# sqeazy/sqeazy

Hardware: AMD Instinct MI355X
Metric: encode GB/s (input voxels) for bitswap1->lz4 uint16 volume (higher is better)
Workload: dtype u16

## Files before the change

sqeazy_amd/csrc/sqy_capi.cpp:

```cpp
#include "../../include/sqeazy_amd.h"

#include <hip/hip_runtime.h>

#include <algorithm>
#include <chrono>
#include <climits>
#include <cstdint>
#include <cstdio>
#include <cstdlib>
#include <cstring>
#include <atomic>
#include <condition_variable>
#include <memory>
#include <mutex>
#include <string>
#include <thread>
#include <vector>

#include "sqy_kernels.h"
#include "sqy_lanes.hpp"
#include "sqy_pipeline.hpp"

namespace {

// ... 17 lines not shown
    const char* v = std::getenv(name);
    if (!v || !*v) return dflt;
    char* end = nullptr;
    const long long x = std::strtoll(v, &end, 10);
    if (*end != '\0' || x < lo || x > hi) {
        std::fprintf(stderr, "[sqeazy]\t %s=%s is not a number in [%ld, %ld]: ignored\n", name, v, lo, hi);
        return dflt;
    }
    return (long)x;
}
constexpr long kWarmupMax = 1l << 30;
constexpr long kStageLanesDefault = 2, kParseLanesDefault = 3;
constexpr long kBatchBytesMax = (1l << 32) - 1, kBatchGroupBytesDefault = 1l << 30;
constexpr long kBatchJointMaxDefault = 128l << 20;
struct Options {
    std::atomic<long> transpose_chain;
    std::atomic<long> transpose_chain_caller_streams;
    std::atomic<long> block_parallel;
    std::atomic<long> block_parallel_warmup;
    std::atomic<long> block_parallel_stats;
    std::atomic<long> tail_scan;
    std::atomic<long> decode_two_waves;
    std::atomic<long> noise_digest;
    std::atomic<long> transpose_blocks_per_cu;
    std::atomic<long> stored_tail_index;
    std::atomic<long> host_l2_bytes;
    std::atomic<long> decode_frames_subset;
    std::atomic<long> decode_slabs_joint;
    std::atomic<long> encode_batch_joint;
    std::atomic<long> encode_batch_group_bytes;
    std::atomic<long> encode_batch_joint_max_bytes;
    std::atomic<long> stage_lanes;
    std::atomic<long> parse_lanes;
    std::atomic<long> lane_calls{0}, lane_backlog_fallbacks{0}, lane_blocked_fallbacks{0};
    std::atomic<long> call_stamps{0};
    Options()
        : transpose_chain(env_flag("SQY_NO_TRANSPOSE_CHAIN") ? 0 : 1), transpose_chain_caller_streams(env_flag("SQY_TRANSPOSE_CHAIN_CALLER_STREAMS")),
          block_parallel(env_flag("SQY_NO_BLOCK_PARALLEL") ? 0 : 1), block_parallel_warmup(env_number("SQY_BLOCK_PARALLEL_WARMUP", 65536, 0, kWarmupMax)),
          block_parallel_stats(env_flag("SQY_BLOCK_PARALLEL_STATS")), tail_scan(env_flag("SQY_NO_TAIL_SCAN") ? 0 : 1),
          decode_two_waves(env_flag("SQY_NO_DECODE_TWO_WAVES") ? 0 : 1), noise_digest(env_flag("SQY_NO_NOISE_DIGEST") ? 0 : 1),
          transpose_blocks_per_cu(env_number("SQY_TRANSPOSE_BLOCKS_PER_CU", 32, 1, 64)), stored_tail_index(env_flag("SQY_NO_STORED_TAIL_INDEX") ? 0 : 1),
          host_l2_bytes((long)sqy::host_l2_cache_bytes()), decode_frames_subset(env_flag("SQY_NO_DECODE_FRAMES_SUBSET") ? 0 : 1),
          decode_slabs_joint(env_flag("SQY_NO_DECODE_SLABS_JOINT") ? 0 : 1), encode_batch_joint(env_flag("SQY_NO_ENCODE_BATCH_JOINT") ? 0 : 1),
          encode_batch_group_bytes(env_number("SQY_ENCODE_BATCH_GROUP_BYTES", kBatchGroupBytesDefault, 1, kBatchBytesMax)),
          encode_batch_joint_max_bytes(env_number("SQY_ENCODE_BATCH_JOINT_MAX_BYTES", kBatchJointMaxDefault, 0, kBatchBytesMax)), stage_lanes(env_number("SQY_STAGE_LANES", kStageLanesDefault, 0, 2)),
          parse_lanes(env_number("SQY_PARSE_LANES", kParseLanesDefault, 1, sqy::LanePicker::kMaxLanes)) { sqy::set_bitswap1_blocks_per_cu(transpose_blocks_per_cu.load()); }
    std::atomic<long>* find(const char* name)
    {
        if (!name) return nullptr;
        if (!std::strcmp(name, "transpose_chain")) return &transpose_chain;
        if (!std::strcmp(name, "transpose_chain_caller_streams")) return &transpose_chain_caller_streams;
        if (!std::strcmp(name, "block_parallel")) return &block_parallel;
        if (!std::strcmp(name, "block_parallel_warmup")) return &block_parallel_warmup;
        if (!std::strcmp(name, "block_parallel_stats")) return &block_parallel_stats;
        if (!std::strcmp(name, "tail_scan")) return &tail_scan;
        if (!std::strcmp(name, "decode_two_waves")) return &decode_two_waves;
        if (!std::strcmp(name, "noise_digest")) return &noise_digest;
        if (!std::strcmp(name, "transpose_blocks_per_cu")) return &transpose_blocks_per_cu;
        if (!std::strcmp(name, "stored_tail_index")) return &stored_tail_index;
        if (!std::strcmp(name, "host_l2_bytes")) return &host_l2_bytes;
        if (!std::strcmp(name, "decode_frames_subset")) return &decode_frames_subset;
        if (!std::strcmp(name, "decode_slabs_joint")) return &decode_slabs_joint;
        if (!std::strcmp(name, "encode_batch_joint")) return &encode_batch_joint;
        if (!std::strcmp(name, "encode_batch_group_bytes")) return &encode_batch_group_bytes;
        if (!std::strcmp(name, "encode_batch_joint_max_bytes")) return &encode_batch_joint_max_bytes;
        if (!std::strcmp(name, "stage_lanes")) return &stage_lanes;
        if (!std::strcmp(name, "parse_lanes")) return &parse_lanes;
        if (!std::strcmp(name, "lane_calls")) return &lane_calls;
        if (!std::strcmp(name, "lane_backlog_fallbacks")) return &lane_backlog_fallbacks;
        if (!std::strcmp(name, "lane_blocked_fallbacks")) return &lane_blocked_fallbacks;
        if (!std::strcmp(name, "call_stamps")) return &call_stamps;
        return nullptr;
    }
};
Options g_opt;

struct CallStamps {
    enum { entry, lanes_taken, clear_launched, transpose_launched, parse_queued, sync_returned, returned, kStamps };
    long seq = -1;
    long lane = -1;
    long thread = 0;
    long ns[kStamps] = {};
    void stamp(int i) { ns[i] = (long)std::chrono::duration_cast<std::chrono::nanoseconds>(std::chrono::steady_clock::now().time_since_epoch()).count(); }
};
constexpr size_t kStampRing = 8192;
std::mutex g_stamps_mu;
std::vector<CallStamps> g_stamps;
size_t g_stamps_next = 0;
struct StampScope {
    CallStamps rec;
    const bool on;
    StampScope() : on(g_opt.call_stamps.load(std::memory_order_relaxed) != 0) 
    {
        if (!on) return;
        rec.stamp(CallStamps::entry);
        rec.thread = (long)(std::hash<std::thread::id>()(std::this_thread::get_id()) & 0x7fffffff);
    }
    CallStamps* get() { return on ? &rec : nullptr; }
    ~StampScope()
    {
// ... 109 lines not shown
    {
        if (bytes <= cap) return 0;
        if (p) { hipHostFree(p); p = nullptr; cap = 0; }
        const size_t want = (bytes + ((size_t)1 << 16) - 1) & ~(((size_t)1 << 16) - 1);
        if (hipHostMalloc(&p, want, hipHostMallocDefault) != hipSuccess) {
            std::fprintf(stderr, "[sqeazy]\t unable to allocate %zu bytes of pinned host memory\n", want);
            (void)hipGetLastError();
            p = nullptr;
            return 1;
        }
        cap = want;
        return 0;
    }
    void release() { if (p) hipHostFree(p); p = nullptr; cap = 0; }
};

struct Workspace {
    DevBuf ping, pong, lz4_scratch, csize, frame_off, io_src, io_dst, small, plan, dedupe;
    DevBuf spec;
    DevBuf diff_side;
    DevBuf digest;
    DevBuf bkrd;
    DevBuf subset;
    DevBuf range_full;
    DevBuf slabs_index;
    DevBuf slabs_joint;
    DevBuf slabs_out;
    HostBuf slabs_host;
    DevBuf batch_stream;
    DevBuf batch_scratch;
    DevBuf batch_tables;
    HostBuf batch_host;
    void* pinned = nullptr;
    void release_buffers()
    {
        ping.release(); pong.release(); lz4_scratch.release(); csize.release(); frame_off.release();
        io_src.release(); io_dst.release(); small.release(); plan.release(); dedupe.release(); diff_side.release(); spec.release(); digest.release(); bkrd.release();
        subset.release(); range_full.release(); slabs_index.release(); slabs_joint.release(); slabs_out.release(); slabs_host.release();
        batch_stream.release(); batch_scratch.release(); batch_tables.release(); batch_host.release();
    }
};

struct Stager {
    static constexpr int kLanes = 4;
    static constexpr size_t kSlice = 8u << 20;
    char* pin[kLanes][2] = {};
    hipStream_t st[kLanes] = {};
    hipEvent_t ev[kLanes][2] = {};
    bool ready = false;

    bool init()
    {
        if (ready) return true;
        for (int l = 0; l < kLanes; ++l) {
            if (hipStreamCreateWithFlags(&st[l], hipStreamNonBlocking) != hipSuccess) return false;
            for (int b = 0; b < 2; ++b) {
                if (hipHostMalloc((void**)&pin[l][b], kSlice, hipHostMallocDefault) != hipSuccess) return false;
                if (hipEventCreateWithFlags(&ev[l][b], hipEventDisableTiming) != hipSuccess) return false;
            }
        }
        ready = true;
        return true;
    }
    bool copy(void* dev, void* host, size_t bytes, bool to_device, int device_id)
    {
        if (bytes == 0) return true;
        if (!init()) return false;
        const size_t nslices = (bytes + kSlice - 1) / kSlice;
// ... 219 lines not shown
Lz4Descriptor lz4_descriptor(int block_id)
{
    const unsigned char fd[2] = {0x40, (unsigned char)(block_id << 4)};
    return {fd[0], fd[1], (sqy::xxh32(fd, 2, 0) >> 8) & 0xff};
}

struct EncodeCall {
    Context& cx;
    Workspace* ws;
    std::vector<PendingEvent>* pend;
    hipStream_t stream;
    LaneLease* lanes;
    CallStamps* stamps;
    Pipeline pipe;
    std::vector<uint64_t> dims;
    uint64_t len;
    int elem_size;
    void* d_dst;
    uint64_t dst_capacity;
    long* dstoffset;
    FrameQuery* fq;

    const uint8_t* cur;
    int cur_elem;
    uint64_t cur_len;
    bool use_ping = true;

    struct {
        sqy::Lz4DedupeLayout dedupe;
        sqy::Lz4InplacePlan place;
        uint32_t* digest = nullptr;
        uint32_t digest_stride = 0;
        bool dedupe_cleared = false;
        const uint64_t* frame_map = nullptr;
        uint64_t frame_bytes = 0;
    } prep;
    struct DiffSide { const uint16_t* p = nullptr; uint32_t w = 0, X = 0; } side;
    struct {
        bool on = false;
        int block_id = 0;
        uint64_t total = 0, chunk = 0, nchunks = 0, stride = 0;
        const sqy::Lz4Block* blocks = nullptr;
        const uint32_t* dup_of = nullptr;
        uint64_t* tail_info = nullptr;
        bool inplace_done = false;
        uint64_t blob_at = 0, blob_bytes = 0, payload_bytes = 0;
    } lz4;

    EncodeCall(Context& c, hipStream_t s, Pipeline&& p, std::vector<uint64_t>&& d, uint64_t voxels, int elem, const void* src, void* dst,
               uint64_t capacity, long* offset, FrameQuery* frames, LaneLease* lane_lease, CallStamps* call_stamps)
        : cx(c), ws(&c.ws), pend(&c.pending), stream(s), lanes(lane_lease), stamps(call_stamps), pipe(std::move(p)), dims(std::move(d)), len(voxels), elem_size(elem), d_dst(dst),
          dst_capacity(capacity), dstoffset(offset), fq(frames), cur(static_cast<const uint8_t*>(src)), cur_elem(elem), cur_len(voxels) {}

    uint8_t* next_buf(size_t bytes)
    {
        DevBuf& b = use_ping ? ws->ping : ws->pong;
        use_ping = !use_ping;
        return b.ensure(bytes) ? nullptr : static_cast<uint8_t*>(b.p);
    }
    int produced(const uint8_t* out) { cur = out; return 0; }
    bool is_tail(size_t si) const { return pipe.sink_index >= 0 && (int)si > pipe.sink_index; }
    bool not_3d(const char* scheme) const
    {
        if (dims.size() != 3) std::fprintf(stderr, "[sqeazy::detail::%s::encode] received non-3D shape which is currently unsupported!\n", scheme);
        return dims.size() != 3;
    }
    bool followed_by(size_t si, StageKind k) const { return si + 1 < pipe.stages.size() && pipe.stages[si + 1].kind == k; }
    void stage_shape(size_t si, uint64_t& Z, uint64_t& Y, uint64_t& X) const
    {
        const bool flat = is_tail(si) && cur_len * (uint64_t)cur_elem != len;
        Z = flat ? 1 : dims[0]; Y = flat ? 1 : dims[1]; X = flat ? cur_len : dims[2];
    }

    int take_lanes(std::unique_lock<std::mutex>& lock)
    {
        const long mode = g_opt.stage_lanes.load();
        if (!lanes || mode == 0 || (mode == 2 && !g_opt.transpose_chain_caller_streams.load()) || (stream != nullptr && stream == cx.stream)) return 0;
        int devid = 0;
        if (hipGetDevice(&devid) != hipSuccess || devid < 0 || devid >= kMaxDev) return 0;
        if (!cx.ensure_lane_event()) { std::fprintf(stderr, "[sqeazy]\t no HIP event for the lanes\n"); return 1; }
        const auto deadline = std::chrono::steady_clock::now() + kLaneArrival;
        for (;;) {
            const hipError_t e = hipStreamQuery(stream);
            if (e == hipSuccess) break;
            (void)hipGetLastError();
// ... 66 lines not shown
            SQY_HIP(hipStreamWaitEvent(stream, g_tchain_last[devid], 0));
        g_tchain_when[devid] = now;
        tc.devid = devid;
        return 0;
    }
    int chain_record(TransposeChain& tc)
    {
        if (tc.devid < 0) return 0;
        SQY_HIP(hipEventRecord(cx.t_done, stream));
        g_tchain_last[tc.devid] = cx.t_done;
        tc.lock.unlock();
        return 0;
    }

    int bitswap1_for_lz4(size_t si, std::unique_lock<std::mutex>& lane_lock)
    {
        const sqy::Lz4Params& lz = pipe.stages[si + 1].lz4;
        const sqy::Lz4EncodeLayout lay = sqy::lz4_encode_layout(lz, cur_len * 2, pipe.nthreads);
        const uint64_t words = sqy::bitswap1_piece_hash_words(cur, cur, cur_len);
        prep.dedupe = sqy::lz4_dedupe_layout(lay, words);
        if (!prep.dedupe.total) return 0;
        if (ws->dedupe.ensure(prep.dedupe.total)) return 1;
        const uint64_t hdr_max = sqy::header_pack(elem_size, false, dims, pipe.name(), (uint64_t)INT_MAX).size() + 2;
        prep.place = sqy::lz4_inplace_plan(lay, words, si + 2 == pipe.stages.size(), dstoffset != nullptr,
                                           (unsigned)(reinterpret_cast<uintptr_t>(d_dst) & 15), dst_capacity, hdr_max);
        if (!prep.place.on) return 0;
        if (ws->plan.ensure((lay.nchunks + 1) * sizeof(uint32_t))) return 1;
        const uint32_t dstride = sqy::lz4_noise_digest_words(lz, lay, g_opt.noise_digest.load() != 0, cur_len / 8);
        if (dstride && !ws->digest.ensure(lay.nchunks * (uint64_t)dstride * sizeof(uint32_t), true)) {
            prep.digest = static_cast<uint32_t*>(ws->digest.p);
            prep.digest_stride = dstride;
        }
        if (take_lanes(lane_lock)) return 1;
        SQY_HIP(sqy::launch_lz4_dedupe_clear(ws->dedupe.p, prep.dedupe, static_cast<uint32_t*>(ws->plan.p), stream));
        prep.dedupe_cleared = true;
        if (stamps) stamps->stamp(CallStamps::clear_launched);
        return 0;
    }

    int bitswap1(size_t si)
    {
        std::unique_lock<std::mutex> lane_lock;
        if (cur_elem == 2 && followed_by(si, StageKind::lz4) && bitswap1_for_lz4(si, lane_lock)) return 1;
        const bool inplace = prep.place.on;
        uint8_t* out = inplace ? static_cast<uint8_t*>(d_dst) + prep.place.body0 : next_buf(cur_len * cur_elem);
        if (!out) return 1;
        if (!inplace && (reinterpret_cast<uintptr_t>(out) & 15)) prep.dedupe = sqy::Lz4DedupeLayout();
        uint32_t* ph = prep.dedupe.total ? static_cast<uint32_t*>(ws->dedupe.p) : nullptr;
        const bool on_lanes = lanes && lanes->taken();
        TransposeChain tc;
        if (chain_wait(tc, inplace)) return 1;
        if (cur_elem == 2)
            SQY_TIMED("bitswap1_u16", sqy::launch_bitswap1_u16(reinterpret_cast<const uint16_t*>(cur), reinterpret_cast<uint16_t*>(out), cur_len, stream, ph,
                                                               inplace ? (uint32_t)prep.place.chunk : 0, side.p, side.w, side.X, inplace ? prep.digest : nullptr,
                                                               prep.digest_stride));
        else
            SQY_TIMED("bitswap1_u8", sqy::launch_bitswap1_u8(cur, out, cur_len, stream));
        if (chain_record(tc)) return 1;
        if (stamps) stamps->stamp(CallStamps::transpose_launched);
        if (on_lanes && leave_transpose_lane(lane_lock)) return 1;
        side = DiffSide();
        return produced(out);
    }

    int reorder(size_t si, bool zcurve)
    {
        const char* name = zcurve ? "zcurve_reorder" : "raster_reorder";
// ... 252 lines not shown
                                           prep.dedupe_cleared, fused_dedupe ? &dedupe_args : nullptr));
            lz4.dup_of = reinterpret_cast<const uint32_t*>(static_cast<const uint8_t*>(ws->dedupe.p) + prep.dedupe.dup_at);
            if (fused_dedupe && prep.digest) { dedupe_args.digest = prep.digest; dedupe_args.digest_stride = prep.digest_stride; }
        }
        if (ws->plan.ensure((lz4.nchunks + 1) * sizeof(uint32_t))) return 1;
        uint32_t* d_redo = static_cast<uint32_t*>(ws->plan.p);
        SQY_TIMED("lz4_chunks", sqy::launch_lz4_chunks(cur, lz4.total, (uint32_t)lz4.chunk, static_cast<uint8_t*>(ws->lz4_scratch.p), lz4.stride,
                                                       static_cast<uint32_t*>(ws->csize.p), lz4.nchunks, stream, prep.frame_map, prep.frame_bytes, d_redo,
                                                       fused_dedupe ? nullptr : lz4.dup_of, prep.place.in_stride, accel, prep.dedupe_cleared,
                                                       fused_dedupe ? &dedupe_args : nullptr));
        std::string hdr_prefix, hdr_suffix;
        if (prep.place.on && !(fq && fq->every > 0)) sqy::header_pack_parts(elem_size, false, dims, pipe.name(), &hdr_prefix, &hdr_suffix);
        if (prep.place.on && !hdr_prefix.empty() && hdr_prefix.size() + hdr_suffix.size() <= sqy::kLz4InplaceHeaderTextMax)
            return lz4_inplace_finish(d_redo, hdr_prefix, hdr_suffix);
        SQY_HIP(hipMemcpyAsync(ws->pinned, d_redo, sizeof(uint32_t), hipMemcpyDeviceToHost, stream));
        SQY_HIP(hipStreamSynchronize(stream));
        const uint32_t n_redo = *static_cast<uint32_t*>(ws->pinned);
        return n_redo ? lz4_dense(d_redo, n_redo) : 0;
    }

    int lz4_dense(uint32_t* d_redo, uint32_t n_redo)
    {
        SQY_TIMED("lz4_chunks_dense", sqy::launch_lz4_chunks_dense(cur, lz4.total, (uint32_t)lz4.chunk, static_cast<uint8_t*>(ws->lz4_scratch.p), lz4.stride,
                                                                   static_cast<uint32_t*>(ws->csize.p), d_redo, n_redo, stream, prep.frame_map, prep.frame_bytes,
                                                                   prep.place.in_stride));
        return 0;
    }

    int lz4_inplace_finish(uint32_t* d_redo, const std::string& hdr_prefix, const std::string& hdr_suffix)
    {
        const Lz4Descriptor fd = lz4_descriptor(lz4.block_id);
        uint8_t* outb = static_cast<uint8_t*>(d_dst);
        volatile uint64_t* record = static_cast<volatile uint64_t*>(ws->pinned);
        const bool fused_tail = lz4.nchunks <= 65536;
        auto tail = [&](const uint32_t* guard, bool fused, bool scan_too) -> int {
            record[0] = 0;
            if (!fused && scan_too)
                SQY_TIMED("lz4_frame_scan", sqy::launch_lz4_frame_scan(static_cast<uint32_t*>(ws->csize.p), lz4.nchunks, lz4.total, (uint32_t)lz4.chunk,
                                                                       static_cast<uint64_t*>(ws->frame_off.p), stream, nullptr, lz4.dup_of, lz4.tail_info, guard,
                                                                       outb + prep.place.body0, prep.place.in_stride, fd.bd, fd.hc));
            auto with_args = [&](auto launch) {
                return launch(outb, prep.place.t0, prep.place.in_stride, lz4.total, (uint32_t)lz4.chunk, lz4.nchunks, static_cast<uint8_t*>(ws->lz4_scratch.p), lz4.stride,
                              static_cast<uint32_t*>(ws->csize.p), static_cast<uint64_t*>(ws->frame_off.p), lz4.dup_of, lz4.tail_info, fd.bd, fd.hc,
                              hdr_prefix.data(), (uint32_t)hdr_prefix.size(), hdr_suffix.data(), (uint32_t)hdr_suffix.size(), (uint32_t)elem_size, guard,
                              const_cast<uint64_t*>(record), stream);
            };
            SQY_TIMED(fused ? "lz4_inplace_tail" : "lz4_frame_gather",
                      fused ? with_args(sqy::launch_lz4_inplace_tail_fused) : with_args(sqy::launch_lz4_inplace_tail));
            return 0;
        };
        if (tail(d_redo, fused_tail, true)) return 1;
        if (stamps) stamps->stamp(CallStamps::parse_queued);
        SQY_HIP(hipStreamSynchronize(stream));
        if (stamps) stamps->stamp(CallStamps::sync_returned);
        if (record[0] == 2) {
            if (lz4_dense(d_redo, (uint32_t)record[6])) return 1;
            if (tail(nullptr, fused_tail, true)) return 1;
            SQY_HIP(hipStreamSynchronize(stream));
        }
        if (record[0] == 4) {
            if (tail(nullptr, false, false)) return 1;
            SQY_HIP(hipStreamSynchronize(stream));
        }
        if (record[0] != 1) {
            std::fprintf(stderr, "[sqeazy]\t internal error: frames in place did not finish (status %llu)\n", (unsigned long long)record[0]);
            return 1;
        }
        lz4.inplace_done = true;
        lz4.blob_at = record[1]; lz4.blob_bytes = record[2]; lz4.payload_bytes = record[3];
        lz4.on = true;
        return 0;
    }

    int lz4_linked(size_t si, bool serial, uint32_t accel)
    {
        const sqy::Lz4Plan plan = sqy::lz4_plan_blocks(lz4.total, lz4.chunk, pipe.stages[si].lz4.block_bytes(), serial);
        if (!plan.ok || plan.blocks.empty()) {
            std::fprintf(stderr, "[sqeazy]\t lz4: block layout not available on MI355X\n");
            return 1;
        }
        const uint64_t nblocks = plan.blocks.size(), nframes = plan.frame_first.size() - 1;
        const uint64_t blocks_bytes = nblocks * sizeof(sqy::Lz4Block), first_bytes = (nframes + 1) * sizeof(uint32_t);
        static_assert(sizeof(sqy::Lz4Block) == sizeof(sqy::Lz4BlockPlan) && sizeof(sqy::Lz4Block) == 32, "plan entries are read by the kernels as they are");
        if (ws->plan.ensure(blocks_bytes + first_bytes)) return 1;
        sqy::Lz4Block* d_blocks = static_cast<sqy::Lz4Block*>(ws->plan.p);
        uint32_t* d_first = reinterpret_cast<uint32_t*>(static_cast<uint8_t*>(ws->plan.p) + blocks_bytes);
        SQY_HIP(hipMemcpyAsync(d_blocks, plan.blocks.data(), blocks_bytes, hipMemcpyHostToDevice, stream));
// ... 139 lines not shown
        if (tail.j) {
            SQY_TIMED("lz4_frame_gather", sqy::launch_lz4_frame_gather(body0, lz4.total, (uint32_t)lz4.chunk, static_cast<uint8_t*>(ws->lz4_scratch.p), lz4.stride,
                                                                       static_cast<uint32_t*>(ws->csize.p), static_cast<uint64_t*>(ws->frame_off.p), out + payload_at, fd.bd, fd.hc,
                                                                       tail.j, stream, nullptr, 0, nullptr, lz4.dup_of, prep.place.in_stride, tail.raw_head != 0));
        }
        SQY_HIP(hipMemcpyAsync(out + *blob_at, hdr.data(), hdr.size(), hipMemcpyHostToDevice, stream));
        SQY_HIP(hipStreamSynchronize(stream));
        return 0;
    }

    int assemble_plain(const std::string& hdr, uint64_t payload_bytes)
    {
        uint8_t* out = static_cast<uint8_t*>(d_dst);
        const Lz4Descriptor fd = lz4_descriptor(lz4.block_id);
        SQY_HIP(hipMemcpyAsync(out, hdr.data(), hdr.size(), hipMemcpyHostToDevice, stream));
        if (lz4.on && lz4.nchunks == 0) {
            const unsigned char empty[7 + 4] = {0x04, 0x22, 0x4D, 0x18, fd.flg, fd.bd, (unsigned char)fd.hc, 0, 0, 0, 0};
            SQY_HIP(hipMemcpyAsync(out + hdr.size(), empty, sizeof(empty), hipMemcpyHostToDevice, stream));
        } else if (lz4.on) {
            SQY_TIMED("lz4_frame_gather", sqy::launch_lz4_frame_gather(cur, lz4.total, (uint32_t)lz4.chunk, static_cast<uint8_t*>(ws->lz4_scratch.p), lz4.stride,
                                                                       static_cast<uint32_t*>(ws->csize.p), static_cast<uint64_t*>(ws->frame_off.p),
                                                                       out + hdr.size(), fd.bd, fd.hc, lz4.nchunks, stream, prep.frame_map, prep.frame_bytes, lz4.blocks, lz4.dup_of));
        } else {
            SQY_TIMED("payload_copy", hipMemcpyAsync(out + hdr.size(), cur, payload_bytes, hipMemcpyDeviceToDevice, stream));
        }
        SQY_HIP(hipStreamSynchronize(stream));
        return 0;
    }

    int done(uint64_t at, uint64_t bytes, long* dstlength)
    {
        if (lanes) lanes->complete = true;
        if (g_prof_on.load()) prof_collect(*pend);
        if (dstoffset) *dstoffset = (long)at;
        *dstlength = (long)bytes;
        return 0;
    }

    int finish(long* dstlength)
    {
        uint64_t payload_bytes = 0, blob_at = 0;
        StoredTail tail;
        if (payload_size(&payload_bytes, &tail)) return 1;
        if (lz4.inplace_done) return done(lz4.blob_at, lz4.blob_bytes, dstlength);
        const std::string hdr = sqy::header_pack(elem_size, false, dims, pipe.name(), payload_bytes);
        if (fq && fq->every > 0 && frame_offsets(hdr.size(), payload_bytes)) return 1;
        const uint64_t blob_bytes = hdr.size() + payload_bytes;
        if (blob_bytes > dst_capacity) {
            std::fprintf(stderr, "[sqeazy]\t destination buffer too small (%llu > %llu bytes)\n", (unsigned long long)blob_bytes,
                         (unsigned long long)dst_capacity);
            return 1;
        }
        if (prep.place.on ? assemble_inplace(hdr, tail, &blob_at) : assemble_plain(hdr, payload_bytes)) return 1;
        return done(blob_at, blob_bytes, dstlength);
    }
};

bool pipeline_admitted(const std::string& pipeline, int elem_size)
{
    std::string why;
    if (Pipeline::supported(pipeline, elem_size, &why)) return true;
    if (Pipeline::reference_accepts(pipeline)) std::fprintf(stderr, "[sqeazy]\t pipeline %s: %s\n", pipeline.c_str(), why.c_str());
    return false;
}

int admit_pipeline(const std::string& pipeline, int elem_size, int nthreads, Pipeline* pipe)
// ... 1768 lines not shown
```

sqeazy_amd/csrc/sqy_kernels.h:

```cpp
#ifndef SQY_KERNELS_H_
#define SQY_KERNELS_H_

#include <hip/hip_runtime_api.h>
#include <stdint.h>

namespace sqy {

struct Lz4DedupeLayout;

struct Lz4DedupeArgs {
    const uint64_t* chunk_key = nullptr;
    const uint64_t* tab_key = nullptr;
    const uint32_t* tab_val = nullptr;
    uint32_t tab_mask = 0;
    uint32_t* dup_of = nullptr;
    const uint32_t* piece_hash = nullptr;
    const uint64_t* holes_map = nullptr;
    uint64_t nchunks_full = 0;
    const uint32_t* digest = nullptr;
    uint32_t digest_stride = 0;
};
hipError_t launch_bitswap1_u16(const uint16_t* in, uint16_t* out, uint64_t len, hipStream_t stream, uint32_t* piece_hash = nullptr,
                               uint32_t gap_chunk = 0, const uint16_t* side = nullptr, uint32_t side_w = 0, uint32_t X = 0,
                               uint32_t* digest = nullptr, uint32_t digest_stride = 0);
// ... 15 lines not shown
                             uint32_t acceleration = 1,
                             bool redo_is_zero = false,
                             const Lz4DedupeArgs* dedupe = nullptr);
hipError_t launch_lz4_chunks_dense(const uint8_t* in, uint64_t total, uint32_t chunk, uint8_t* scratch, uint64_t stride,
                                   uint32_t* csize, uint32_t* redo, uint32_t redo_count, hipStream_t stream,
                                   const uint64_t* frame_map = nullptr, uint64_t frame_bytes = 0, uint64_t in_stride = 0);
struct Lz4Block {
    uint64_t start;
    uint32_t n;
    uint32_t flags;
    int64_t low_in, low_dict;
};
hipError_t launch_lz4_linked(const uint8_t* in, const Lz4Block* blocks, const uint32_t* frame_first, uint64_t nframes,
                             uint32_t max_block, uint8_t* scratch, uint64_t stride, uint32_t* csize, hipStream_t stream, uint32_t acceleration = 1);
struct Lz4SpecArgs {
    const uint32_t* wave_first = nullptr;
    const uint32_t* wave_last = nullptr;
    uint32_t* tables = nullptr;
    uint32_t mode = 0;
};
constexpr uint64_t kLz4SpecTableWords = 2 * 4096;
hipError_t launch_lz4_linked_spec(const uint8_t* in, const Lz4Block* blocks, const Lz4SpecArgs& spec, uint64_t nwaves,
                                  uint32_t max_block, uint8_t* scratch, uint64_t stride, uint32_t* csize, hipStream_t stream, uint32_t acceleration = 1);
hipError_t launch_lz4_linked_verify(const Lz4Block* blocks, uint64_t nblocks, const uint32_t* tables, uint32_t max_block, uint32_t* ok, hipStream_t stream);
hipError_t launch_lz4_frame_scan(const uint32_t* csize, uint64_t nchunks, uint64_t total, uint32_t chunk,
                                 uint64_t* frame_off, hipStream_t stream, const Lz4Block* blocks = nullptr,
                                 const uint32_t* dup_of = nullptr, uint64_t* tail_info = nullptr,
                                 const uint32_t* guard = nullptr, uint8_t* body0 = nullptr, uint64_t in_stride = 0, uint32_t bd_byte = 0,
                                 uint32_t hc_byte = 0);
hipError_t launch_lz4_inplace_tail_fused(uint8_t* out, uint64_t t0, uint64_t in_stride, uint64_t total, uint32_t chunk, uint64_t nchunks,
                                         const uint8_t* scratch, uint64_t stride, const uint32_t* csize, uint64_t* frame_off, const uint32_t* dup_of,
                                         uint64_t* tail_info, uint32_t bd_byte, uint32_t hc_byte, const char* hdr_prefix, uint32_t prefix_len,
                                         const char* hdr_suffix, uint32_t suffix_len, uint32_t elem_size, const uint32_t* guard, uint64_t* record,
                                         hipStream_t stream);
hipError_t launch_lz4_inplace_tail(uint8_t* out, uint64_t t0, uint64_t in_stride, uint64_t total, uint32_t chunk, uint64_t nchunks,
                                   uint8_t* scratch, uint64_t stride, const uint32_t* csize, const uint64_t* frame_off, const uint32_t* dup_of,
                                   const uint64_t* tail_info, uint32_t bd_byte, uint32_t hc_byte, const char* hdr_prefix, uint32_t prefix_len,
                                   const char* hdr_suffix, uint32_t suffix_len, uint32_t elem_size, const uint32_t* guard, uint64_t* record,
                                   hipStream_t stream);
constexpr uint32_t kLz4InplaceHeaderTextMax = 3000;
hipError_t launch_lz4_tail_marks(uint8_t* body0, uint64_t in_stride, uint64_t total, uint32_t chunk, uint64_t nchunks, uint32_t bd_byte,
                                 uint32_t hc_byte, const uint64_t* tail_info, hipStream_t stream);
hipError_t launch_lz4_stash_raw(const uint8_t* body0, uint64_t in_stride, uint64_t total, uint32_t chunk, uint8_t* scratch, uint64_t stride,
                                const uint32_t* csize, const uint32_t* dup_of, uint64_t nhead, hipStream_t stream);
hipError_t launch_lz4_frame_gather(const uint8_t* in, uint64_t total, uint32_t chunk, const uint8_t* scratch, uint64_t stride,
                                   const uint32_t* csize, const uint64_t* frame_off, uint8_t* out, uint32_t bd_byte,
                                   uint32_t hc_byte, uint64_t nchunks, hipStream_t stream, const uint64_t* frame_map = nullptr,
                                   uint64_t frame_bytes = 0, const Lz4Block* blocks = nullptr, const uint32_t* dup_of = nullptr,
                                   uint64_t in_stride = 0, bool raw_from_scratch = false);

struct Bitswap1Job { const void* in; void* out; uint64_t len; };
uint32_t batch_bitswap1_tiles(uint64_t len);
hipError_t launch_bitswap1_batch(const Bitswap1Job* d_jobs, const uint32_t* d_first_tile, uint32_t njobs, uint32_t ntiles, int elem_size, hipStream_t stream);
struct Lz4BatchChunk { uint64_t off; uint32_t n, vol, slot, pad; };
hipError_t launch_lz4_chunks_table(const uint8_t* in, const Lz4BatchChunk* d_table, uint32_t nentries, uint8_t* scratch, uint64_t stride, uint32_t* csize,
                                   uint32_t* redo, hipStream_t stream);
hipError_t launch_lz4_chunks_table_dense(const uint8_t* in, const Lz4BatchChunk* d_table, uint8_t* scratch, uint64_t stride, uint32_t* csize,
                                         uint32_t* redo, uint32_t redo_count, hipStream_t stream);
struct Lz4BatchVolume { uint64_t dst_at, capacity; uint32_t first_chunk, nchunks, text_at, prefix_len, suffix_len, elem_size, record, pad; };
constexpr uint64_t kBatchDone = 1, kBatchNoRoom = 2, kBatchPayloadTooLong = 3;
hipError_t launch_lz4_batch_scan(const Lz4BatchChunk* d_table, const Lz4BatchVolume* d_vols, uint32_t nvols, const uint32_t* csize,
                                 uint64_t* frame_off, uint64_t* vinfo, hipStream_t stream);
hipError_t launch_lz4_batch_gather(const uint8_t* in, const Lz4BatchChunk* d_table, uint32_t nentries, uint32_t max_chunk, const Lz4BatchVolume* d_vols,
                                   const uint32_t* d_vol_of , const uint8_t* scratch, uint64_t stride,
                                   const uint32_t* csize, const uint64_t* frame_off, const uint64_t* vinfo, const char* d_text, uint8_t* out,
                                   uint32_t bd_byte, uint32_t hc_byte, uint64_t* records, hipStream_t stream);

// ... 80 lines not shown
```

sqeazy_amd/csrc/sqy_kernels.hip:

```cpp
#include <hip/hip_runtime.h>
#include <atomic>
#include <mutex>
#include <stdint.h>
#include <cstring>
#include <type_traits>

#include "sqy_kernels.h"
#include "sqy_pipeline.hpp"

namespace sqy {

struct __attribute__((packed)) pk_u16 { uint16_t v; };
struct __attribute__((packed)) pk_u32 { uint32_t v; };
struct __attribute__((packed)) pk_u64 { uint64_t v; };
struct __attribute__((packed)) pk_u128 { uint32_t x, y, z, w; };

__device__ __forceinline__ uint32_t ld_u32(const uint8_t* p) { return reinterpret_cast<const pk_u32*>(p)->v; }
__device__ __forceinline__ uint64_t ld_u64(const uint8_t* p) { return reinterpret_cast<const pk_u64*>(p)->v; }
__device__ __forceinline__ uint4 ld_u128(const uint8_t* p)
{
    const pk_u128 t = *reinterpret_cast<const pk_u128*>(p);
    return make_uint4(t.x, t.y, t.z, t.w);
}
__device__ __forceinline__ void st_u32(uint8_t* p, uint32_t v) { reinterpret_cast<pk_u32*>(p)->v = v; }
// ... 5544 lines not shown
            const uint32_t pp = e >> tsh;
            const uint32_t e2 = pp >= n_prev ? (((pp - n_prev) << tsh) | (e & tmask)) : 0u;
            d |= e2 ^ used[i];
        }
        if (d) differ = 1;
    }
    __syncthreads();
    if (threadIdx.x == 0) ok[k] = differ ? 0u : 1u;
}

hipError_t launch_lz4_linked_verify(const Lz4Block* blocks, uint64_t nblocks, const uint32_t* tables, uint32_t max_block, uint32_t* ok, hipStream_t stream)
{
    if (nblocks == 0) return hipSuccess;
    if (max_block == 0 || max_block > (4u << 20)) return hipErrorInvalidValue;
    hipLaunchKernelGGL(lz4_linked_verify_kernel, dim3((unsigned)nblocks), dim3(256), 0, stream, blocks, tables, max_block, ok);
    return hipGetLastError();
}

hipError_t launch_lz4_frame_scan(const uint32_t* csize, uint64_t nchunks, uint64_t total, uint32_t chunk,
                                 uint64_t* frame_off, hipStream_t stream, const Lz4Block* blocks, const uint32_t* dup_of, uint64_t* tail_info,
                                 const uint32_t* guard, uint8_t* body0, uint64_t in_stride, uint32_t bd_byte, uint32_t hc_byte)
{
    hipLaunchKernelGGL(lz4_frame_scan_kernel, dim3(1), dim3(256), 0, stream, csize, nchunks, total, chunk, frame_off, blocks, dup_of, tail_info,
                       guard, body0, in_stride, bd_byte, hc_byte);
    return hipGetLastError();
}

constexpr uint32_t TAIL_THREADS = 64;
__global__ __launch_bounds__(TAIL_THREADS)
void lz4_inplace_tail_fused_kernel(uint8_t* __restrict__ out, uint64_t t0, uint64_t in_stride, uint64_t total, uint32_t chunk, uint64_t nchunks,
                                   uint32_t cpb, const uint8_t* __restrict__ scratch, uint64_t stride, const uint32_t* __restrict__ csize,
                                   uint64_t* __restrict__ frame_off, const uint32_t* __restrict__ dup_of, uint64_t* __restrict__ tail_info,
                                   uint32_t bd_byte, uint32_t hc_byte, Lz4HeaderParts hp, uint32_t elem_size, const uint32_t* __restrict__ guard,
                                   uint64_t* __restrict__ record)
{
    const uint32_t tid = threadIdx.x, lane = tid & 63u, wave = tid >> 6;
    if (guard && guard[0] != 0u) {
        if (blockIdx.x == 0 && tid == 0) { record[6] = guard[0]; record[0] = 2; }
        return;
    }
    __shared__ uint64_t red_sum[TAIL_THREADS / 64], red_before[TAIL_THREADS / 64];
    __shared__ uint32_t red_j[TAIL_THREADS / 64], red_zero[TAIL_THREADS / 64];
    __shared__ uint64_t own_off[64];
    __shared__ uint32_t own_c[64], own_ks[64];
    const uint64_t k_first = (uint64_t)blockIdx.x * cpb;
    uint64_t sum = 0, before = 0;
    uint32_t jmax = 0, nzero = 0;
    for (uint64_t base = 0; base < nchunks; base += TAIL_THREADS * 8u) {
        uint32_t ks[8], c[8];
#pragma unroll
        for (uint32_t u = 0; u < 8; ++u) {
            const uint64_t k = base + u * TAIL_THREADS + tid;
            ks[u] = k < nchunks ? (dup_of ? dup_of[k] : (uint32_t)k) : 0u;
        }
#pragma unroll
        for (uint32_t u = 0; u < 8; ++u) {
            const uint64_t k = base + u * TAIL_THREADS + tid;
            c[u] = k < nchunks ? csize[ks[u]] : 0u;
        }
#pragma unroll
        for (uint32_t u = 0; u < 8; ++u) {
            const uint64_t k = base + u * TAIL_THREADS + tid;
            if (k < nchunks) {
                const uint64_t left = total - k * chunk;
                const uint64_t nk = left < chunk ? left : chunk;
                const uint64_t sz = 15u + (c[u] ? c[u] : nk);
                sum += sz;
                if (k < k_first) before += sz;
                if (c[u]) jmax = jmax > (uint32_t)k + 1u ? jmax : (uint32_t)k + 1u; else nzero += 1u;
                if (k >= k_first && k < k_first + cpb) { own_c[k - k_first] = c[u]; own_ks[k - k_first] = ks[u]; }
            }
        }
    }
// ... 94 lines not shown
        do { digits[nd++] = (char)('0' + v % 10); v /= 10; } while (v);
    }
    const uint64_t text = (uint64_t)hp.prefix_len + nd + hp.suffix_len;
    const uint64_t pad = (elem_size - text % elem_size) % elem_size;
    const uint64_t hdr_len = text + pad;
    if (hdr_len > payload_at) {
        if (tid == 0) record[0] = 3;
        return;
    }
    uint8_t* h = out + payload_at - hdr_len;
    for (uint64_t i = tid; i < hdr_len; i += TAIL_THREADS) {
        uint8_t cch;
        if (i < pad) cch = ' ';
        else if (i < pad + hp.prefix_len) cch = (uint8_t)hp.text[i - pad];
        else if (i < pad + hp.prefix_len + nd) cch = (uint8_t)digits[nd - 1 - (i - pad - hp.prefix_len)];
        else cch = (uint8_t)hp.text[hp.prefix_len + (i - pad - hp.prefix_len - nd)];
        h[i] = cch;
    }
    if (tid == 0) {
        record[1] = payload_at - hdr_len;
        record[2] = hdr_len + payload;
        record[3] = payload;
        record[4] = j;
        record[5] = 0;
        record[6] = 0;
        record[0] = 1;
    }
}

hipError_t launch_lz4_inplace_tail_fused(uint8_t* out, uint64_t t0, uint64_t in_stride, uint64_t total, uint32_t chunk, uint64_t nchunks,
                                         const uint8_t* scratch, uint64_t stride, const uint32_t* csize, uint64_t* frame_off, const uint32_t* dup_of,
                                         uint64_t* tail_info, uint32_t bd_byte, uint32_t hc_byte, const char* hdr_prefix, uint32_t prefix_len,
                                         const char* hdr_suffix, uint32_t suffix_len, uint32_t elem_size, const uint32_t* guard, uint64_t* record,
                                         hipStream_t stream)
{
    Lz4HeaderParts hp;
    if ((uint64_t)prefix_len + suffix_len > sizeof(hp.text) || nchunks == 0 || nchunks > 0x7fffffffull) return hipErrorInvalidValue;
    hp.prefix_len = prefix_len; hp.suffix_len = suffix_len;
    std::memcpy(hp.text, hdr_prefix, prefix_len);
    std::memcpy(hp.text + prefix_len, hdr_suffix, suffix_len);
    uint32_t cpb = (uint32_t)((nchunks + 1023u) / 1024u);
    if (cpb < 4u) cpb = 4u;
    if (cpb > 64u) return hipErrorInvalidValue;
    const unsigned grid = (unsigned)((nchunks + cpb - 1u) / cpb);
    hipLaunchKernelGGL(lz4_inplace_tail_fused_kernel, dim3(grid), dim3(TAIL_THREADS), 0, stream, out, t0, in_stride, total, chunk, nchunks, cpb, scratch,
                       stride, csize, frame_off, dup_of, tail_info, bd_byte, hc_byte, hp, elem_size, guard, record);
    return hipGetLastError();
}

hipError_t launch_lz4_inplace_tail(uint8_t* out, uint64_t t0, uint64_t in_stride, uint64_t total, uint32_t chunk, uint64_t nchunks,
                                   uint8_t* scratch, uint64_t stride, const uint32_t* csize, const uint64_t* frame_off, const uint32_t* dup_of,
                                   const uint64_t* tail_info, uint32_t bd_byte, uint32_t hc_byte, const char* hdr_prefix, uint32_t prefix_len,
                                   const char* hdr_suffix, uint32_t suffix_len, uint32_t elem_size, const uint32_t* guard, uint64_t* record,
                                   hipStream_t stream)
{
    Lz4HeaderParts hp;
    if ((uint64_t)prefix_len + suffix_len > sizeof(hp.text) || nchunks == 0) return hipErrorInvalidValue;
    hp.prefix_len = prefix_len; hp.suffix_len = suffix_len;
    std::memcpy(hp.text, hdr_prefix, prefix_len);
    std::memcpy(hp.text + prefix_len, hdr_suffix, suffix_len);
    uint8_t* body0 = out + t0 + kLz4FrameHead;
    const uint32_t slices_stash = (chunk + 32767u) / 32768u, slices = (chunk + GATHER_SLICE - 1) / GATHER_SLICE;
    const uint64_t stash_items = nchunks * slices_stash, gather_items = nchunks * slices;
    hipLaunchKernelGGL(lz4_stash_raw_kernel, dim3((unsigned)(stash_items < 1024 ? stash_items : 1024)), dim3(256), 0, stream, body0, in_stride, total, chunk,
                       scratch, stride, csize, dup_of, slices_stash, tail_info, guard);
    hipLaunchKernelGGL(lz4_frame_gather_kernel, dim3((unsigned)(gather_items < 2048 ? gather_items : 2048)), dim3(256), 0, stream, body0, total, chunk,
                       scratch, stride, csize, frame_off, out, bd_byte, hc_byte, slices, (const uint64_t*)nullptr, (uint64_t)0, (const Lz4Block*)nullptr,
                       dup_of, in_stride, 0, tail_info, t0, guard);
    hipLaunchKernelGGL(lz4_inplace_finish_kernel, dim3(1), dim3(256), 0, stream, out, t0, in_stride, tail_info, hp, elem_size, guard, record);
    return hipGetLastError();
}

hipError_t launch_lz4_tail_marks(uint8_t* body0, uint64_t in_stride, uint64_t total, uint32_t chunk, uint64_t nchunks, uint32_t bd_byte,
                                 uint32_t hc_byte, const uint64_t* tail_info, hipStream_t stream)
{
    if (nchunks == 0) return hipSuccess;
    hipLaunchKernelGGL(lz4_tail_marks_kernel, dim3((unsigned)((nchunks + 255) / 256)), dim3(256), 0, stream, body0, in_stride, total, chunk,
                       nchunks, bd_byte, hc_byte, tail_info);
    return hipGetLastError();
// ... 962 lines not shown
```

sqeazy_amd/csrc/sqy_pipeline.cpp:

```cpp
#include "sqy_pipeline.hpp"

#pragma clang fp contract(off)

#include <algorithm>
#include <cerrno>
#include <climits>
#include <cmath>
#include <cstdint>
#include <cstdio>
#include <cstdlib>
#include <cstring>
#include <sstream>
#include <sys/stat.h>
#include <thread>
#if defined(__x86_64__) || defined(__i386__)
#include <cpuid.h>
#endif

namespace sqy {

const char* const kVersion = "0.5.2";
const char* const kHeadRef = "mi355x";
const int kVersionTriple[3] = {0, 5, 2};

// ... 278 lines not shown
        group_sum += total;
        plan.group_of[i] = (int32_t)(plan.groups.size() - 1);
    }
    return plan;
}

Lz4DedupeLayout lz4_dedupe_layout(const Lz4EncodeLayout& lay, uint64_t piece_hash_words)
{
    Lz4DedupeLayout d;
    if (!piece_hash_words || !lay.chunked() || lay.chunk % 1024 != 0 || lay.nchunks < 2) return d;
    d.table = 64;
    while (d.table < 2 * lay.nchunks) d.table <<= 1;
    d.work_at = round_up(piece_hash_words * 4, 64);
    d.tab_key_at = d.work_at + lay.nchunks * 8;
    d.tab_val_at = d.tab_key_at + d.table * 8;
    d.dup_at = d.tab_val_at + d.table * 4 + 64;
    d.holes_at = d.dup_at + round_up(lay.nchunks * 4, 8);
    d.total = d.holes_at + lay.nchunks * (1u + ((lay.chunk >> 10) + 63u) / 64u) * 8u;
    return d;
}

Lz4InplacePlan lz4_inplace_plan(const Lz4EncodeLayout& lay, uint64_t piece_hash_words, bool lz4_is_last, bool takes_offset, unsigned dst_mod16,
                                uint64_t capacity, uint64_t header_max)
{
    Lz4InplacePlan p;
    if (!lz4_dedupe_layout(lay, piece_hash_words).total || !lz4_is_last || !takes_offset || (lay.chunk & (lay.chunk - 1))) return p;
    p.chunk = lay.chunk;
    p.t0 = header_max;
    while ((dst_mod16 + p.t0 + kLz4FrameHead) & 15) ++p.t0;
    p.in_stride = lay.chunk + kLz4FrameGap;
    p.body0 = p.t0 + kLz4FrameHead;
    p.on = p.t0 + lay.nchunks * p.in_stride <= capacity;
    return p.on ? p : Lz4InplacePlan();
}

static uint32_t lz4_noise_digest_stride(uint32_t chunk)
{
    if (chunk < 16384u || (chunk & (chunk - 1u))) return 0;
    uint64_t p = 1, st = 1, nb = 64, probes = 0;
    for (;;) {
        ++probes;
        const uint64_t p2 = p + st;
        st = nb >> 6; ++nb;
        if (p2 > (uint64_t)chunk - 12 + 1) break;
        p = p2;
    }
    if (probes <= 961) return 0;
    return (uint32_t)(((probes - 960) + 63) & ~(uint64_t)63);
}

uint32_t lz4_noise_digest_words(const Lz4Params& p, const Lz4EncodeLayout& lay, bool option_on, uint64_t segment_bytes)
{
    const uint32_t stride = lay.chunk <= 0xffffffffull ? lz4_noise_digest_stride((uint32_t)lay.chunk) : 0;
    return option_on && stride && segment_bytes % lay.chunk == 0 && p.accel >= 0 ? stride : 0;
}

bool lz4_spec_wanted(const Lz4Plan& plan)
{
    const uint64_t nframes = plan.frame_first.size() - 1;
    uint64_t longest = 0;
    for (uint64_t f = 0; f < nframes; ++f) longest = std::max<uint64_t>(longest, plan.frame_first[f + 1] - plan.frame_first[f]);
    return longest >= 3 && nframes < 1024;
}

void lz4_warmup_windows(const Lz4Plan& plan, uint64_t warmup, std::vector<uint32_t>* first, std::vector<uint32_t>* last)
{
// ... 841 lines not shown
```

sqeazy_amd/csrc/sqy_pipeline.hpp:

```cpp
#ifndef SQY_PIPELINE_HPP_
#define SQY_PIPELINE_HPP_

#include <cstdint>
#include <map>
#include <string>
#include <utility>
#include <vector>

namespace sqy {

typedef std::vector<std::pair<std::string, std::string>> pairs_t;

std::vector<std::string> split_outside_verbatim(const std::string& s, const std::string& sep, bool* ok = nullptr);
pairs_t parse_pairs(const std::string& pipeline);
std::map<std::string, std::string> parse_minors(const std::string& cfg);

enum class StageKind { diff3x3x1, bitswap1, bitshuffle, frame_shuffle, raster_reorder, zcurve_reorder, tile_shuffle, quantiser, lz4, pass_through,
                       rmestbkrd, rmbkrd_neighbor5, unsupported };

struct Lz4Params {
    int accel = 1;
    uint32_t blocksize_kb = 256, framestep_kb = 256, n_chunks = 0;
    int block_id = 5;
    explicit Lz4Params(const std::string& cfg = "");
// ... 27 lines not shown
};
Lz4EncodeLayout lz4_encode_layout(const Lz4Params& p, uint64_t total, unsigned nthreads);

struct Lz4BatchChunkPlan {
    uint64_t off;
    uint32_t n;
    uint32_t vol;
    uint32_t slot;
    uint32_t pad = 0;
};
struct Lz4BatchGroup {
    std::vector<uint32_t> vols;
    std::vector<uint64_t> stream_at;
    std::vector<uint32_t> first_chunk;
    std::vector<Lz4BatchChunkPlan> chunks;
    uint64_t stream_bytes = 0;
    uint64_t scratch_stride = 0;
    uint32_t max_chunk = 0;
};
struct Lz4BatchPlan {
    std::vector<int32_t> group_of;
    std::vector<Lz4BatchGroup> groups;
};
Lz4BatchPlan lz4_batch_plan(const Lz4Params& p, const std::vector<uint64_t>& totals, unsigned nthreads, uint64_t group_bytes, uint64_t joint_max);

constexpr uint64_t kLz4FrameHead = 7 + 4, kLz4FrameGap = kLz4FrameHead + 4;
struct Lz4InplacePlan { bool on = false; uint64_t chunk = 0, t0 = 0, in_stride = 0, body0 = 0; };
Lz4InplacePlan lz4_inplace_plan(const Lz4EncodeLayout& lay, uint64_t piece_hash_words, bool lz4_is_last, bool takes_offset, unsigned dst_mod16,
                                uint64_t capacity, uint64_t header_max);
uint32_t lz4_noise_digest_words(const Lz4Params& p, const Lz4EncodeLayout& lay, bool option_on, uint64_t segment_bytes);

struct Lz4DedupeLayout { uint64_t table = 0, work_at = 0, tab_key_at = 0, tab_val_at = 0, dup_at = 0, holes_at = 0, total = 0; };
Lz4DedupeLayout lz4_dedupe_layout(const Lz4EncodeLayout& lay, uint64_t piece_hash_words);

bool lz4_spec_wanted(const Lz4Plan& plan);
void lz4_warmup_windows(const Lz4Plan& plan, uint64_t warmup, std::vector<uint32_t>* first, std::vector<uint32_t>* last);
struct Lz4RedoRuns { uint64_t nruns = 0, longest = 0; };
Lz4RedoRuns lz4_redo_runs(const Lz4Plan& plan, const std::vector<uint32_t>& ok, uint64_t run_max, std::vector<uint32_t>* first, std::vector<uint32_t>* last);

struct Lz4DecodeGeometry { uint64_t chunk = 1, nchunks = 0, block_bytes = 0, max_blocks = 0; };
Lz4DecodeGeometry lz4_decode_geometry(const Lz4Params& p, uint64_t total);
bool lz4_chunks_whole(uint64_t nframes, uint64_t nchunks, uint64_t total, uint64_t chunk);
bool lz4_folds_into_shuffle(uint64_t nframes, uint64_t nchunks, uint64_t total, uint64_t chunk, uint64_t Z, uint64_t fb);
bool frame_shuffle_decode_map(std::vector<unsigned char>* map, uint64_t Z, std::vector<uint64_t>* unnamed, bool* permutation);

enum class RangeForm { plain, planes, planes_lut, shuffle };
struct FrameRangePlan {
    bool ok = false;
    std::vector<uint32_t> ids;
    uint64_t out_bytes = 0;
    uint64_t range_at = 0;
    std::vector<uint64_t> coff;
    uint64_t plane[16] = {}, tail = 0, v0 = 0, v1 = 0, w0 = 0, w1 = 0, L = 0;
    int we = 1;
    std::vector<uint64_t> remap;
    uint64_t pa = 0, pb = 0;
    bool direct = false;
    std::vector<std::pair<uint64_t, uint64_t>> zero_runs;
};
FrameRangePlan frame_range_plan(RangeForm form, uint64_t n, int elem, uint64_t shape0, uint64_t z0, uint64_t nz, uint64_t chunk, uint64_t total,
                                uint32_t nframes, const std::vector<unsigned char>& struck_map = {}, uint64_t place_bytes = 0, uint64_t places = 0);

struct Stage {
    std::string name;
    StageKind kind = StageKind::unsupported;
    std::map<std::string, std::string> cfg;
// ... 79 lines not shown
```

Measured before the change: 2141.

## Fold dedupe table clearing into fused LZ4 tail kernel for next call

Instead of launching a separate dedupe-table clear kernel at the start of each encode, the fused in-place tail kernel now zeroes the dedupe hash table after finishing, and the workspace records that the table is clean. The next encode call skips the clear launch when the table base, size and counter match and the previous tail finished with status 1. This removes one kernel launch per encode, bringing the count to three. It adds cross-call state that must stay consistent with the buffers, and it makes the tail kernel do extra writes.

```diff
diff --git a/sqeazy_amd/csrc/sqy_capi.cpp b/sqeazy_amd/csrc/sqy_capi.cpp
--- a/sqeazy_amd/csrc/sqy_capi.cpp
+++ b/sqeazy_amd/csrc/sqy_capi.cpp
@@ -73,6 +73,7 @@
     std::atomic<long> encode_batch_joint_max_bytes;
     std::atomic<long> stage_lanes;
     std::atomic<long> parse_lanes;
+    std::atomic<long> encode_three_launches;
     std::atomic<long> lane_calls{0}, lane_backlog_fallbacks{0}, lane_blocked_fallbacks{0};
     std::atomic<long> call_stamps{0};
     Options()
@@ -85,7 +86,8 @@
           decode_slabs_joint(env_flag("SQY_NO_DECODE_SLABS_JOINT") ? 0 : 1), encode_batch_joint(env_flag("SQY_NO_ENCODE_BATCH_JOINT") ? 0 : 1),
           encode_batch_group_bytes(env_number("SQY_ENCODE_BATCH_GROUP_BYTES", kBatchGroupBytesDefault, 1, kBatchBytesMax)),
           encode_batch_joint_max_bytes(env_number("SQY_ENCODE_BATCH_JOINT_MAX_BYTES", kBatchJointMaxDefault, 0, kBatchBytesMax)), stage_lanes(env_number("SQY_STAGE_LANES", kStageLanesDefault, 0, 2)),
-          parse_lanes(env_number("SQY_PARSE_LANES", kParseLanesDefault, 1, sqy::LanePicker::kMaxLanes)) { sqy::set_bitswap1_blocks_per_cu(transpose_blocks_per_cu.load()); }
+          parse_lanes(env_number("SQY_PARSE_LANES", kParseLanesDefault, 1, sqy::LanePicker::kMaxLanes)),
+          encode_three_launches(env_flag("SQY_NO_ENCODE_THREE_LAUNCHES") ? 0 : 1) { sqy::set_bitswap1_blocks_per_cu(transpose_blocks_per_cu.load()); }
     std::atomic<long>* find(const char* name)
     {
         if (!name) return nullptr;
@@ -107,6 +109,7 @@
         if (!std::strcmp(name, "encode_batch_joint_max_bytes")) return &encode_batch_joint_max_bytes;
         if (!std::strcmp(name, "stage_lanes")) return &stage_lanes;
         if (!std::strcmp(name, "parse_lanes")) return &parse_lanes;
+        if (!std::strcmp(name, "encode_three_launches")) return &encode_three_launches;
         if (!std::strcmp(name, "lane_calls")) return &lane_calls;
         if (!std::strcmp(name, "lane_backlog_fallbacks")) return &lane_backlog_fallbacks;
         if (!std::strcmp(name, "lane_blocked_fallbacks")) return &lane_blocked_fallbacks;
@@ -282,8 +285,10 @@
     DevBuf batch_tables;
     HostBuf batch_host;
     void* pinned = nullptr;
+    sqy::Lz4DedupeState dedupe_state;
     void release_buffers()
     {
+        dedupe_state = sqy::Lz4DedupeState();
         ping.release(); pong.release(); lz4_scratch.release(); csize.release(); frame_off.release();
         io_src.release(); io_dst.release(); small.release(); plan.release(); dedupe.release(); diff_side.release(); spec.release(); digest.release(); bkrd.release();
         subset.release(); range_full.release(); slabs_index.release(); slabs_joint.release(); slabs_out.release(); slabs_host.release();
@@ -569,6 +574,8 @@
         uint32_t* digest = nullptr;
         uint32_t digest_stride = 0;
         bool dedupe_cleared = false;
+        sqy::Lz4CleanPlan clean;
+        uint64_t first_tail_status = 0;
         const uint64_t* frame_map = nullptr;
         uint64_t frame_bytes = 0;
     } prep;
@@ -587,7 +594,10 @@
     EncodeCall(Context& c, hipStream_t s, Pipeline&& p, std::vector<uint64_t>&& d, uint64_t voxels, int elem, const void* src, void* dst,
                uint64_t capacity, long* offset, FrameQuery* frames, LaneLease* lane_lease, CallStamps* call_stamps)
         : cx(c), ws(&c.ws), pend(&c.pending), stream(s), lanes(lane_lease), stamps(call_stamps), pipe(std::move(p)), dims(std::move(d)), len(voxels), elem_size(elem), d_dst(dst),
-          dst_capacity(capacity), dstoffset(offset), fq(frames), cur(static_cast<const uint8_t*>(src)), cur_elem(elem), cur_len(voxels) {}
+          dst_capacity(capacity), dstoffset(offset), fq(frames), cur(static_cast<const uint8_t*>(src)), cur_elem(elem), cur_len(voxels),
+          dedupe_before(sqy::lz4_dedupe_state_take(&c.ws.dedupe_state)) {}
+    const sqy::Lz4DedupeState dedupe_before;
+    const void* dedupe_table() const { return static_cast<const uint8_t*>(ws->dedupe.p) + prep.dedupe.tab_key_at; }
 
     uint8_t* next_buf(size_t bytes)
     {
@@ -720,7 +730,8 @@
             prep.digest_stride = dstride;
         }
         if (take_lanes(lane_lock)) return 1;
-        SQY_HIP(sqy::launch_lz4_dedupe_clear(ws->dedupe.p, prep.dedupe, static_cast<uint32_t*>(ws->plan.p), stream));
+        prep.clean = sqy::lz4_clean_plan(g_opt.encode_three_launches.load() != 0, true, lay.nchunks, prep.dedupe, dedupe_table(), ws->plan.p, dedupe_before);
+        if (prep.clean.clear_first) SQY_TIMED("lz4_dedupe_clear", sqy::launch_lz4_dedupe_clear(ws->dedupe.p, prep.dedupe, static_cast<uint32_t*>(ws->plan.p), stream));
         prep.dedupe_cleared = true;
         if (stamps) stamps->stamp(CallStamps::clear_launched);
         return 0;
@@ -1039,7 +1050,7 @@
         const Lz4Descriptor fd = lz4_descriptor(lz4.block_id);
         uint8_t* outb = static_cast<uint8_t*>(d_dst);
         volatile uint64_t* record = static_cast<volatile uint64_t*>(ws->pinned);
-        const bool fused_tail = lz4.nchunks <= 65536;
+        const bool fused_tail = lz4.nchunks <= sqy::kLz4FusedTailChunksMax;
         auto tail = [&](const uint32_t* guard, bool fused, bool scan_too) -> int {
             record[0] = 0;
             if (!fused && scan_too)
@@ -1052,14 +1063,17 @@
                               hdr_prefix.data(), (uint32_t)hdr_prefix.size(), hdr_suffix.data(), (uint32_t)hdr_suffix.size(), (uint32_t)elem_size, guard,
                               const_cast<uint64_t*>(record), stream);
             };
-            SQY_TIMED(fused ? "lz4_inplace_tail" : "lz4_frame_gather",
-                      fused ? with_args(sqy::launch_lz4_inplace_tail_fused) : with_args(sqy::launch_lz4_inplace_tail));
+            auto fused_and_clean = [&](auto... a) {
+                return sqy::launch_lz4_inplace_tail_fused(a..., prep.clean.tail_cleans ? ws->dedupe.p : nullptr, &prep.dedupe);
+            };
+            SQY_TIMED(fused ? "lz4_inplace_tail" : "lz4_frame_gather", fused ? with_args(fused_and_clean) : with_args(sqy::launch_lz4_inplace_tail));
             return 0;
         };
         if (tail(d_redo, fused_tail, true)) return 1;
         if (stamps) stamps->stamp(CallStamps::parse_queued);
         SQY_HIP(hipStreamSynchronize(stream));
         if (stamps) stamps->stamp(CallStamps::sync_returned);
+        prep.first_tail_status = fused_tail ? record[0] : 0;
         if (record[0] == 2) {
             if (lz4_dense(d_redo, (uint32_t)record[6])) return 1;
             if (tail(nullptr, fused_tail, true)) return 1;
@@ -1265,6 +1279,7 @@
     {
         if (lanes) lanes->complete = true;
         if (g_prof_on.load()) prof_collect(*pend);
+        if (prep.clean.tail_cleans) ws->dedupe_state = sqy::lz4_dedupe_state_after(prep.clean, prep.dedupe, dedupe_table(), ws->plan.p, prep.first_tail_status, true);
         if (dstoffset) *dstoffset = (long)at;
         *dstlength = (long)bytes;
         return 0;
diff --git a/sqeazy_amd/csrc/sqy_kernels.h b/sqeazy_amd/csrc/sqy_kernels.h
--- a/sqeazy_amd/csrc/sqy_kernels.h
+++ b/sqeazy_amd/csrc/sqy_kernels.h
@@ -71,7 +71,8 @@
                                          const uint8_t* scratch, uint64_t stride, const uint32_t* csize, uint64_t* frame_off, const uint32_t* dup_of,
                                          uint64_t* tail_info, uint32_t bd_byte, uint32_t hc_byte, const char* hdr_prefix, uint32_t prefix_len,
                                          const char* hdr_suffix, uint32_t suffix_len, uint32_t elem_size, const uint32_t* guard, uint64_t* record,
-                                         hipStream_t stream);
+                                         hipStream_t stream,
+                                         void* clean_base = nullptr, const Lz4DedupeLayout* clean_lay = nullptr);
 hipError_t launch_lz4_inplace_tail(uint8_t* out, uint64_t t0, uint64_t in_stride, uint64_t total, uint32_t chunk, uint64_t nchunks,
                                    uint8_t* scratch, uint64_t stride, const uint32_t* csize, const uint64_t* frame_off, const uint32_t* dup_of,
                                    const uint64_t* tail_info, uint32_t bd_byte, uint32_t hc_byte, const char* hdr_prefix, uint32_t prefix_len,
diff --git a/sqeazy_amd/csrc/sqy_kernels.hip b/sqeazy_amd/csrc/sqy_kernels.hip
--- a/sqeazy_amd/csrc/sqy_kernels.hip
+++ b/sqeazy_amd/csrc/sqy_kernels.hip
@@ -5600,13 +5600,15 @@
                                    uint32_t cpb, const uint8_t* __restrict__ scratch, uint64_t stride, const uint32_t* __restrict__ csize,
                                    uint64_t* __restrict__ frame_off, const uint32_t* __restrict__ dup_of, uint64_t* __restrict__ tail_info,
                                    uint32_t bd_byte, uint32_t hc_byte, Lz4HeaderParts hp, uint32_t elem_size, const uint32_t* __restrict__ guard,
-                                   uint64_t* __restrict__ record)
+                                   uint64_t* __restrict__ record, uint64_t* __restrict__ clean_key, uint32_t* __restrict__ clean_val, uint32_t clean_tab)
 {
     const uint32_t tid = threadIdx.x, lane = tid & 63u, wave = tid >> 6;
     if (guard && guard[0] != 0u) {
         if (blockIdx.x == 0 && tid == 0) { record[6] = guard[0]; record[0] = 2; }
         return;
     }
+    if (clean_key)
+        for (uint32_t i = blockIdx.x * TAIL_THREADS + tid; i < clean_tab; i += gridDim.x * TAIL_THREADS) { clean_key[i] = 0ull; clean_val[i] = 0xffffffffu; }
     __shared__ uint64_t red_sum[TAIL_THREADS / 64], red_before[TAIL_THREADS / 64];
     __shared__ uint32_t red_j[TAIL_THREADS / 64], red_zero[TAIL_THREADS / 64];
     __shared__ uint64_t own_off[64];
@@ -5767,7 +5769,7 @@
                                          const uint8_t* scratch, uint64_t stride, const uint32_t* csize, uint64_t* frame_off, const uint32_t* dup_of,
                                          uint64_t* tail_info, uint32_t bd_byte, uint32_t hc_byte, const char* hdr_prefix, uint32_t prefix_len,
                                          const char* hdr_suffix, uint32_t suffix_len, uint32_t elem_size, const uint32_t* guard, uint64_t* record,
-                                         hipStream_t stream)
+                                         hipStream_t stream, void* clean_base, const Lz4DedupeLayout* clean_lay)
 {
     Lz4HeaderParts hp;
     if ((uint64_t)prefix_len + suffix_len > sizeof(hp.text) || nchunks == 0 || nchunks > 0x7fffffffull) return hipErrorInvalidValue;
@@ -5778,8 +5780,12 @@
     if (cpb < 4u) cpb = 4u;
     if (cpb > 64u) return hipErrorInvalidValue;
     const unsigned grid = (unsigned)((nchunks + cpb - 1u) / cpb);
+    const bool clean = clean_base && clean_lay && clean_lay->total && guard;
+    uint64_t* clean_key = clean ? reinterpret_cast<uint64_t*>(static_cast<uint8_t*>(clean_base) + clean_lay->tab_key_at) : nullptr;
+    uint32_t* clean_val = clean ? reinterpret_cast<uint32_t*>(static_cast<uint8_t*>(clean_base) + clean_lay->tab_val_at) : nullptr;
+    const uint32_t clean_tab = clean ? (uint32_t)clean_lay->table : 0u;
     hipLaunchKernelGGL(lz4_inplace_tail_fused_kernel, dim3(grid), dim3(TAIL_THREADS), 0, stream, out, t0, in_stride, total, chunk, nchunks, cpb, scratch,
-                       stride, csize, frame_off, dup_of, tail_info, bd_byte, hc_byte, hp, elem_size, guard, record);
+                       stride, csize, frame_off, dup_of, tail_info, bd_byte, hc_byte, hp, elem_size, guard, record, clean_key, clean_val, clean_tab);
     return hipGetLastError();
 }
 
diff --git a/sqeazy_amd/csrc/sqy_pipeline.cpp b/sqeazy_amd/csrc/sqy_pipeline.cpp
--- a/sqeazy_amd/csrc/sqy_pipeline.cpp
+++ b/sqeazy_amd/csrc/sqy_pipeline.cpp
@@ -334,6 +334,25 @@
     p.body0 = p.t0 + kLz4FrameHead;
     p.on = p.t0 + lay.nchunks * p.in_stride <= capacity;
     return p.on ? p : Lz4InplacePlan();
+}
+
+Lz4CleanPlan lz4_clean_plan(bool option_on, bool inplace, uint64_t nchunks, const Lz4DedupeLayout& d, const void* table_base, const void* counter,
+                            const Lz4DedupeState& before)
+{
+    Lz4CleanPlan p;
+    if (!d.total || !table_base || !counter) return p;
+    p.tail_cleans = option_on && inplace && nchunks <= kLz4FusedTailChunksMax;
+    p.clear_first = !(option_on && inplace && before.clean && before.table == d.table && before.table_base == table_base && before.counter == counter);
+    return p;
+}
+
+Lz4DedupeState lz4_dedupe_state_after(const Lz4CleanPlan& plan, const Lz4DedupeLayout& d, const void* table_base, const void* counter,
+                                      uint64_t first_tail_status, bool success)
+{
+    Lz4DedupeState s;
+    if (!plan.tail_cleans || !success || first_tail_status != 1 || !d.total) return s;
+    s.clean = true; s.table = d.table; s.table_base = table_base; s.counter = counter;
+    return s;
 }
 
 static uint32_t lz4_noise_digest_stride(uint32_t chunk)
diff --git a/sqeazy_amd/csrc/sqy_pipeline.hpp b/sqeazy_amd/csrc/sqy_pipeline.hpp
--- a/sqeazy_amd/csrc/sqy_pipeline.hpp
+++ b/sqeazy_amd/csrc/sqy_pipeline.hpp
@@ -83,6 +83,15 @@
 
 struct Lz4DedupeLayout { uint64_t table = 0, work_at = 0, tab_key_at = 0, tab_val_at = 0, dup_at = 0, holes_at = 0, total = 0; };
 Lz4DedupeLayout lz4_dedupe_layout(const Lz4EncodeLayout& lay, uint64_t piece_hash_words);
+
+struct Lz4DedupeState { bool clean = false; uint64_t table = 0; const void* table_base = nullptr; const void* counter = nullptr; };
+inline Lz4DedupeState lz4_dedupe_state_take(Lz4DedupeState* of_context) { const Lz4DedupeState s = *of_context; *of_context = Lz4DedupeState(); return s; }
+struct Lz4CleanPlan { bool clear_first = true, tail_cleans = false; };
+Lz4CleanPlan lz4_clean_plan(bool option_on, bool inplace, uint64_t nchunks, const Lz4DedupeLayout& d, const void* table_base, const void* counter,
+                            const Lz4DedupeState& before);
+constexpr uint64_t kLz4FusedTailChunksMax = 65536;
+Lz4DedupeState lz4_dedupe_state_after(const Lz4CleanPlan& plan, const Lz4DedupeLayout& d, const void* table_base, const void* counter,
+                                      uint64_t first_tail_status, bool success);
 
 bool lz4_spec_wanted(const Lz4Plan& plan);
 void lz4_warmup_windows(const Lz4Plan& plan, uint64_t warmup, std::vector<uint32_t>* first, std::vector<uint32_t>* last);
```

Result: slower. 2071 (-3.3%).
